# wtaylor17/ImageCFGen-Pytorch

Hardware: AMD Instinct MI355X
Metric: ALI training images/sec (E+G+D step), MorphoMNIST bs=512/GPU (higher is better)
Workload: dtype f32; 1 GPU; image_scms/mnist.py ALI iteration (EG step + 2 D steps + diagnostics), MorphoMNIST 28x28x1 synthetic, bs=512/GPU, fp32 MFMA, mode=stepper+hipgraph; global_batch=512, parallelism=dp1

## Files before the change

imagecfgen-pytorch_amd/csrc/ali_common.h:

```cpp
#pragma once
#include <hip/hip_runtime.h>
#include <stdint.h>
#include <stdio.h>
#include <stdlib.h>
#include "../../include/ali_hip.h"

namespace ali {

void set_error(const char* fmt, ...);

inline int check_launch(const char* what) {
  hipError_t e = hipGetLastError();
  if (e != hipSuccess) {
    set_error("%s: %s", what, hipGetErrorString(e));
    return ALI_ERR_LAUNCH;
  }
  return ALI_OK;
}

struct Tuning {
  int bm, bn, splitk;
  long long wgrad_small;
  int wgrad_blocks, wgrad_scap;
  int no_first_wgrad;
  int no_order;
  int tile_m_scale;
  int wbm, wbn;
  int no_xcd;
  int no_s2_first;
  int no_dma16;
  int no_t1_mfma;
};
inline Tuning read_tuning() {
  {
    auto num = [](const char* name) -> long long { const char* e = getenv(name); return e ? atoll(e) : 0; };
    Tuning v;
    v.bm = (int)num("ALI_BM"); v.bn = (int)num("ALI_BN"); v.splitk = (int)num("ALI_SPLITK");
    v.wgrad_small = getenv("ALI_WGRAD_SMALL") ? num("ALI_WGRAD_SMALL") : -1;
    v.wgrad_blocks = (int)num("ALI_WGRAD_BLOCKS"); v.wgrad_scap = (int)num("ALI_WGRAD_SCAP");
    v.no_order = (int)num("ALI_NO_ORDER");
    v.no_first_wgrad = (int)num("ALI_NO_FIRST_WGRAD");
    v.tile_m_scale = (int)num("ALI_TILE_M_SCALE");
    v.wbm = (int)num("ALI_WBM"); v.wbn = (int)num("ALI_WBN");
    v.no_t1_mfma = (int)num("ALI_NO_T1_MFMA");
    v.no_xcd = (int)num("ALI_NO_XCD");
    v.no_s2_first = (int)num("ALI_NO_S2_FIRST");
    v.no_dma16 = (int)num("ALI_NO_DMA16");
    return v;
  }
}
inline Tuning& tuning_slot() {
  static Tuning t = read_tuning();
  return t;
}
inline const Tuning& tuning() { return tuning_slot(); }

using f32x4 = __attribute__((ext_vector_type(4))) float;
using f32x16 = __attribute__((ext_vector_type(16))) float;

constexpr int kMaxTaps = 28;
constexpr int kNumCU = 256;

constexpr size_t kWsReserved = ALI_WS_RESERVED;
inline void* ws_payload(void* ws) { return ws ? static_cast<char*>(ws) + kWsReserved : nullptr; }
inline size_t ws_payload_bytes(size_t bytes) { return bytes > kWsReserved ? bytes - kWsReserved : 0; }

__device__ __forceinline__ float apply_act(float v, int act, float slope) {
  if (act == ALI_ACT_LEAKY) return v > 0.f ? v : v * slope;
  if (act == ALI_ACT_TANH) return tanhf(v);
  return v;
}
__device__ __forceinline__ float act_grad_from_output(float y, int act, float slope) {
  if (act == ALI_ACT_LEAKY) return y > 0.f ? 1.f : slope;
  if (act == ALI_ACT_TANH) return 1.f - y * y;
  return 1.f;
}

}
```

imagecfgen-pytorch_amd/csrc/gconv.hip:

```cpp
#include "ali_common.h"
#include <algorithm>
#include <vector>
#include <stdarg.h>
#include <stdlib.h>
#include <string.h>
#include <type_traits>

namespace ali {

static thread_local char g_err[512] = "";
void set_error(const char* fmt, ...) {
  va_list ap;
  va_start(ap, fmt);
  vsnprintf(g_err, sizeof(g_err), fmt, ap);
  va_end(ap);
}
const char* get_error() { return g_err; }

constexpr int BK = 32;
constexpr int LDK = BK + 4;
constexpr int kMaxGrid = 5;

struct Phase {
  int Hq, Wq;
// ... 959 lines not shown
      for (int pix = m_lo / d.B; pix <= m_hi / d.B; ++pix) {
        const int qh = pix / P.Wq, qw = pix - qh * P.Wq;
        unsigned wbits = 0u;
        for (int is = 0; is < P.ns; ++is)
          if ((unsigned)(qw * P.mult + P.dw[is]) < (unsigned)d.Win) wbits |= 1u << is;
        for (int ir = 0; ir < P.nr; ++ir)
          if ((unsigned)(qh * P.mult + P.dh[ir]) < (unsigned)d.Hin) mask |= wbits << (ir * P.ns);
      }
      cost.push_back(__builtin_popcount(mask));
    }
  }
  return true;
}

struct GJobRec {
  uint64_t state;
  int variant;
  int gx, gy, gz;
  int cost;
  GDesc d;
};
static_assert(sizeof(GJobRec) <= sizeof(AliGemmJob), "AliGemmJob too small");

static int finalize_and_launch(GDesc& d, void* ws, size_t ws_bytes, hipStream_t stream, bool vec, bool dense_k,
                               AliGemmJob* job = nullptr) {
  TileCfg tc;
  int max_taps = 0;
  const bool uni = vec && (d.Cin % BK) == 0;
  const bool dma_ok = d.f16 && uni && d.in16 && d.w16 && (d.Cin % 64) == 0 && !d.ep.bn_part && d.ep.in_ld <= 0 &&
                      tuning().no_dma16 == 0 && tuning().splitk == 0;
  const int tiles = plan_tiles(d, vec, tc, max_taps, dma_ok);
  if (tiles < 0) return ALI_ERR_BAD_ARG;
  const bool dma = tc.bm == 256;
  const int max_nkt = (max_taps * d.Cin + BK - 1) / BK;
  const bool pow2 = vec && (d.Cin == 4 || d.Cin == 8 || d.Cin == 16) && max_taps <= kMaxTaps;
  if (d.ep.bn_part) {
    const AliEpilogue& e = d.ep;
    bool ok = (e.bn_mode == 1 || e.bn_mode == 2) && !e.dact_y;
    if (e.bn_mode == 2) ok = ok && !e.mask && e.bn_x && e.bn_mean && e.bn_invstd && e.bn_groups <= 1;
    if (e.bn_mode == 1 && e.bn_groups > 1) {
      ok = ok && d.nphase == 1 && d.B % e.bn_groups == 0;
      const long long rows_g = (long long)(d.B / e.bn_groups) * (d.ph[0].pixmajor ? 1 : d.ph[0].Hq * d.ph[0].Wq);
      ok = ok && rows_g % tc.bm == 0 && (!d.ph[0].pixmajor || d.B % tc.bm == 0);
    }
    if (!ok) { set_error("gconv: bad fused BatchNorm epilogue (see AliEpilogue / ali_conv_mtiles)"); return ALI_ERR_BAD_ARG; }
    if (e.bn_slots > 0 && e.bn_slots != tiles) {
      set_error("gconv: bn_part was sized for %d slots, this launch has %d M-tiles (stale ali_conv_mtiles result?)", e.bn_slots, tiles);
      return ALI_ERR_BAD_ARG;
    }
  }
  const int ntile_n = (d.Cout + tc.bn - 1) / tc.bn;
  d.ldi = d.Cin;
  if (d.ep.in_ld > 0 || d.ep.out_ld > 0) {
    if ((d.ep.in_ld > 0 && (d.ep.in_ld < d.Cin || (vec && d.ep.in_ld % 4))) ||
        (d.ep.out_ld > 0 && (d.ep.out_ld < d.Cout || d.ep.bn_part))) {
      set_error("gconv: bad in_ld / out_ld (>= the channel count, in_ld % 4 == 0 for vector gathers, no out_ld with fused BatchNorm)");
      return ALI_ERR_BAD_ARG;
    }
    if (d.ep.in_ld > 0) d.ldi = d.ep.in_ld;
    if (d.ep.out_ld > 0) d.ldo = d.ep.out_ld;
  }
  d.out_elems = (long long)d.B * d.Hout * d.Wout * d.ldo;
  const long long in_elems = ((long long)d.B * d.Hin * d.Win - 1) * d.ldi + d.Cin;
  const long long w_elems = (long long)d.Cout * d.ldw;
  if (d.out_elems >= (1LL << 31) || in_elems >= (1LL << 30) || w_elems >= (1LL << 29)) {
    set_error("gconv: tensor too large for 32-bit byte offsets");
    return ALI_ERR_BAD_ARG;
  }
  d.in_bytes = (unsigned)(in_elems * 4);
  d.w_bytes = (unsigned)(w_elems * 4);
  int S = 1;
  const long long blocks = (long long)tiles * ntile_n;
  if (blocks < 2 * kNumCU && max_nkt >= 8 && dense_k) {
    static const double eff[5] = {1.0, 0.82, 0.96, 0.99, 1.0};
    double best = 1e30;
    for (int sc = 1; sc <= 8 && max_nkt / sc >= 4; ++sc) {
      if (sc > 1 && (size_t)sc * d.out_elems * sizeof(float) > ws_payload_bytes(ws_bytes)) break;
      const long long n = (blocks * sc + kNumCU - 1) / kNumCU;
      const double cost = (double)n / sc / eff[n < 4 ? n : 4] * max_nkt + (sc > 1 ? 0.5 * sc : 0.0);
      if (cost < 0.97 * best) { best = cost; S = sc; }
    }
  } else if (blocks < 2 * kNumCU && max_nkt >= 8) {
    S = (int)((2 * kNumCU + blocks - 1) / blocks);
    if (S > max_nkt / 4) S = max_nkt / 4;
    if (S > 32) S = 32;
    while (S > 1 && (size_t)S * d.out_elems * sizeof(float) > ws_payload_bytes(ws_bytes)) --S;
    if (S < 1) S = 1;
  }
  if (tuning().splitk > 0 && (size_t)tuning().splitk * d.out_elems * sizeof(float) <= ws_payload_bytes(ws_bytes))
    S = tuning().splitk;
  if (dma) S = 1;
  if (blocks > (long long)(kWsReserved / sizeof(int)) || !ws) S = 1;
  while (S > 1 && (long long)S * d.out_elems * 4 >= 0xFF000000LL) --S;
  d.splitk = S;
  d.kt_per_split = (max_nkt + S - 1) / S;
  if (d.kt_per_split < 1) d.kt_per_split = 1;
  d.ntile_m = tiles;
  d.ntile_n = ntile_n;
  d.tail_split = 1;
  d.tail_u0 = 0;
  if (S == 1 && uni && ws && blocks > kNumCU && blocks < 4 * kNumCU && blocks <= (long long)(kWsReserved / sizeof(int))
      && tuning().splitk == 0 && !dma) {
    const int R = (int)(blocks % kNumCU);
    int Sr = 1;
    while (R > 0 && Sr * 2 <= 8 && Sr * 2 * R <= kNumCU && max_nkt / (Sr * 2) >= 4) Sr *= 2;
    if (Sr > 1 && (size_t)Sr * d.out_elems * sizeof(float) <= ws_payload_bytes(ws_bytes) &&
        (long long)Sr * d.out_elems * 4 < 0xFF000000LL) {
      d.tail_split = Sr;
      d.tail_u0 = (int)(blocks - R);
    }
  }
  d.order = nullptr;
  if (d.ep.tile_order && uni && S == 1 && d.ep.tile_order_n == tiles && tuning().no_order == 0)
    d.order = reinterpret_cast<const int*>(d.ep.tile_order);
  d.lin1d = (d.tail_split > 1 || d.order) ? 1 : 0;
  if (d.tail_split == 1) d.tail_u0 = (int)blocks;
  d.xcd_chunk = 0;
  bool img_major = d.nphase >= 1;
  for (int i = 0; i < d.nphase; ++i) img_major = img_major && !d.ph[i].pixmajor;
  if (!d.lin1d && S == 1 && !job && img_major && blocks >= 8LL * kNumCU && blocks < (1LL << 30) && tuning().no_xcd == 0) {
    d.xcd_chunk = (int)((blocks + 7) / 8);
    d.lin1d = 1;
  }
  d.ctr = reinterpret_cast<int*>(ws);
  d.ws = reinterpret_cast<float*>(ws_payload(ws));
  dim3 grid(tiles, ntile_n, S), block(256);
  if (d.lin1d) grid = dim3(d.tail_u0 + (int)(blocks - d.tail_u0) * d.tail_split, 1, 1);
  if (d.xcd_chunk) grid = dim3(8 * d.xcd_chunk, 1, 1);
  if (tiles == 0 || d.out_elems == 0) return ALI_OK;
  const bool f16 = d.f16 && uni;
  const bool op16 = f16 && d.in16 && d.w16 && (d.Cin % 64) == 0;
  if (!d.f16) d.out16 = nullptr;
  if (job && uni && !f16 && ((tc.bm == 64 && tc.bn == 64) || (tc.bm == 128 && tc.bn == 32))) {
    GJobRec r;
    memset(&r, 0, sizeof(r));
    r.state = 1;
    r.variant = tc.bm == 64 ? 0 : 1;
    r.gx = (int)grid.x; r.gy = (int)grid.y; r.gz = (int)grid.z;
    r.cost = (max_nkt + S - 1) / S;
    r.d = d;
    memcpy(job, &r, sizeof(r));
    return ALI_OK;
  }
#define LAUNCH(BM_, BN_, WMM, WNN)                                                                    \
  do {                                                                                                  \
    if (op16) hipLaunchKernelGGL((gconv_kernel<BM_, BN_, WMM, WNN, 2, 2>), grid, block, 0, stream, d);  \
    else if (f16) hipLaunchKernelGGL((gconv_kernel<BM_, BN_, WMM, WNN, 2, 1>), grid, block, 0, stream, d); \
    else if (uni) hipLaunchKernelGGL((gconv_kernel<BM_, BN_, WMM, WNN, 2>), grid, block, 0, stream, d); \
    else if (pow2) hipLaunchKernelGGL((gconv_kernel<BM_, BN_, WMM, WNN, 3>), grid, block, 0, stream, d);  \
    else if (vec) hipLaunchKernelGGL((gconv_kernel<BM_, BN_, WMM, WNN, 1>), grid, block, 0, stream, d); \
    else hipLaunchKernelGGL((gconv_kernel<BM_, BN_, WMM, WNN, 0>), grid, block, 0, stream, d);          \
  } while (0)
  if (dma) {
    if (tc.bn != 256 || !op16) { set_error("gconv: no kernel for this tile"); return ALI_ERR_BAD_ARG; }
    block = dim3(512);
    hipLaunchKernelGGL((gconv_kernel512<256, 256, 2, 4, 2, 3>), grid, block, 0, stream, d);
    return check_launch("gconv_kernel512");
  }
  if (tc.bm > 128 || tc.bn > 128) { set_error("gconv: no kernel for this tile"); return ALI_ERR_BAD_ARG; }
  else if (tc.bm == 128 && tc.bn == 128) LAUNCH(128, 128, 2, 2);
  else if (tc.bm == 128 && tc.bn == 64) LAUNCH(128, 64, 2, 2);
  else if (tc.bm == 128 && tc.bn == 32) LAUNCH(128, 32, 4, 1);
  else if (tc.bm == 64 && tc.bn == 128) LAUNCH(64, 128, 2, 2);
  else LAUNCH(64, 64, 2, 2);
#undef LAUNCH
  return check_launch("gconv_kernel");
}

static bool geom_ok(const AliConvGeom* g) {
  if (!g) return false;
  if (g->B <= 0 || g->H <= 0 || g->W <= 0 || g->C <= 0 || g->P <= 0 || g->Q <= 0 || g->K <= 0) return false;
  if (g->R <= 0 || g->S <= 0 || g->R > kMaxGrid || g->S > kMaxGrid || g->stride <= 0 || g->pad < 0) return false;
  if (g->pad > 100) return false;
  return true;
}

static void fill_epilogue(GDesc& d, const AliEpilogue* ep) {
  if (ep) d.ep = *ep;
  else memset(&d.ep, 0, sizeof(d.ep));
  d.f16 = d.ep.mfma_f16 != 0;
  d.in16 = reinterpret_cast<const _Float16*>(d.ep.in16);
  d.w16 = reinterpret_cast<const _Float16*>(d.ep.w16);
  d.out16 = reinterpret_cast<_Float16*>(d.ep.out16);
}

}

using namespace ali;

extern "C" const char* ali_last_error(void) { return ali::get_error(); }
extern "C" int ali_version(void) { return 1; }
extern "C" void ali_reload_tuning(void) { ali::tuning_slot() = ali::read_tuning(); }

extern "C" size_t ali_conv_workspace_bytes(const AliConvGeom* g, int32_t which) {
  if (!geom_ok(g)) return 0;
  if (which == 0) return kWsReserved + (size_t)32 * g->B * g->P * g->Q * g->K * sizeof(float);
  if (which == 1) return kWsReserved + (size_t)32 * g->B * g->H * g->W * g->C * sizeof(float);
  return kWsReserved + (size_t)64 * g->R * g->S * g->C * g->K * sizeof(float);
}


constexpr int CF_C = 8, CF_K = 32;
constexpr int CF_PIXLD = 12;

struct CFDesc {
  const float* in; const float* w; float* out;
  AliEpilogue ep;
  int B, H, W, P, Q, R, S;
};

template <int TAPS, int CL = 8>
__global__ __launch_bounds__(256) void conv_first_kernel(const CFDesc d) {
  extern __shared__ __attribute__((aligned(16))) float cf_smem[];
  float* img = cf_smem;
  float* red = cf_smem + d.H * d.W * CF_PIXLD;
  const float* wl = d.w;
  const int t = threadIdx.x, lane = t & 63, wave = t >> 6;
  const int b = blockIdx.x;
  const int HW = d.H * d.W, PQ = d.P * d.Q;
  const float* src = d.in + (long long)b * HW * CF_C;
  for (int i = t; i < HW * 2; i += 256) {
    const f32x4 v = *reinterpret_cast<const f32x4*>(src + i * 4);
    *reinterpret_cast<f32x4*>(img + (i >> 1) * CF_PIXLD + (i & 1) * 4) = v;
  }
  const int lrow = lane & 31, lh = lane >> 5;
  constexpr int CF_WLD = TAPS * CF_C;
  constexpr int KL = TAPS * CL, NS = (KL + 1) / 2;
  f32x4 wf[CL == 8 ? TAPS : 1];
  float wb[CL == 8 ? 1 : NS];
  int aoff[CL == 8 ? 1 : NS];
  if constexpr (CL == 8) {
#pragma unroll
    for (int tp = 0; tp < TAPS; ++tp) wf[tp] = *reinterpret_cast<const f32x4*>(wl + lrow * CF_WLD + tp * CF_C + lh * 4);
  } else {
#pragma unroll
    for (int st = 0; st < NS; ++st) {
      const int k = 2 * st + lh;
      const bool live = k < KL;
      const int kk = live ? k : KL - 1;
      const int tp = kk / CL, c = kk - tp * CL;
      const int r = tp / d.S, sx = tp - r * d.S;
      wb[st] = live ? wl[lrow * CF_WLD + tp * CF_C + c] : 0.f;
      aoff[st] = (r * d.W + sx) * CF_PIXLD + c;
    }
  }
  __syncthreads();
  const AliEpilogue& ep = d.ep;
  const float bias = ep.bias ? ep.bias[lrow] : 0.f;
  const float smask = (ep.bn_part && ep.bn_stat_mask) ? ep.bn_stat_mask[(long long)b * ep.bn_mask_ld + lrow] : 1.f;
  float bs0 = 0.f, bs1 = 0.f;
  const int ntile = (PQ + 31) / 32;
  float* outb = d.out + (long long)b * PQ * CF_K;
  for (int mt = wave; mt < ntile; mt += 4) {
    const int m = mt * 32 + lrow;
    const int mc = m < PQ ? m : PQ - 1;
    const int p = mc / d.Q, q = mc - p * d.Q;
    f32x16 acc;
#pragma unroll
    for (int r = 0; r < 16; ++r) acc[r] = 0.f;
    if constexpr (CL == 8) {
      const float* a0 = img + (p * d.W + q) * CF_PIXLD + lh * 4;
#pragma unroll
      for (int tp = 0; tp < TAPS; ++tp) {
        const int r = tp / d.S, sx = tp - r * d.S;
        const f32x4 av = *reinterpret_cast<const f32x4*>(a0 + (r * d.W + sx) * CF_PIXLD);
#pragma unroll
        for (int e = 0; e < 4; ++e) acc = __builtin_amdgcn_mfma_f32_32x32x2f32(av[e], wf[tp][e], acc, 0, 0, 0);
      }
    } else {
      const float* a0 = img + (p * d.W + q) * CF_PIXLD;
#pragma unroll
      for (int st = 0; st < NS; ++st) {
        float av = a0[aoff[st]];
        if ((KL & 1) && st == NS - 1 && lh) av = 0.f;
        acc = __builtin_amdgcn_mfma_f32_32x32x2f32(av, wb[st], acc, 0, 0, 0);
      }
    }
#pragma unroll
    for (int r = 0; r < 16; ++r) {
      const int row = mt * 32 + (r & 3) + 8 * (r >> 2) + 4 * lh;
      if (row < PQ) {
        const float v = apply_act(acc[r] + bias, ep.act, ep.slope);
        outb[(long long)row * CF_K + lrow] = v;
        const float vs = v * smask;
        bs0 += vs;
        bs1 += vs * vs;
      }
    }
  }
  if (ep.bn_part) {
    bs0 += __shfl_xor(bs0, 32, 64);
    bs1 += __shfl_xor(bs1, 32, 64);
    if (lane < 32) { red[(0 * 4 + wave) * 32 + lane] = bs0; red[(1 * 4 + wave) * 32 + lane] = bs1; }
    __syncthreads();
    if (t < 32) {
      const float a = ((red[t] + red[32 + t]) + red[64 + t]) + red[96 + t];
      const float c = ((red[128 + t] + red[160 + t]) + red[192 + t]) + red[224 + t];
      ep.bn_part[((long long)0 * CF_K + t) * d.B + b] = a;
      ep.bn_part[((long long)1 * CF_K + t) * d.B + b] = c;
    }
  }
}

static bool conv_first_ok(const AliConvGeom* g, const AliEpilogue* ep, bool f16) {
  if (g->C != CF_C || g->K != CF_K || g->stride != 1 || g->pad != 0 || g->R != g->S || (g->R != 5 && g->R != 3)) return false;
  if (g->H > 32 || g->W > 32 || g->B < 64 || f16) return false;
  if (g->P != g->H - g->R + 1 || g->Q != g->W - g->S + 1) return false;
  if (ep && (ep->mask || ep->dact_y || (ep->bn_part && ep->bn_mode != 1))) return false;
  if (ep && ep->bn_part && ep->bn_groups > 1 && g->B % ep->bn_groups != 0) return false;
  return true;
}

static int conv_first_launch(const AliConvGeom* g, const float* x, const float* w, float* y, const AliEpilogue* ep,
                             hipStream_t stream) {
  CFDesc d;
  memset(&d, 0, sizeof(d));
  d.in = x; d.w = w; d.out = y;
  if (ep) d.ep = *ep;
  d.B = g->B; d.H = g->H; d.W = g->W; d.P = g->P; d.Q = g->Q; d.R = g->R; d.S = g->S;
  const size_t lds = ((size_t)g->H * g->W * CF_PIXLD + 256) * sizeof(float);
  const int live = ep ? ep->in_ch_live : 0;
  if (g->R == 5 && live == 5) hipLaunchKernelGGL((conv_first_kernel<25, 5>), dim3(g->B), dim3(256), lds, stream, d);
  else if (g->R == 5) hipLaunchKernelGGL((conv_first_kernel<25>), dim3(g->B), dim3(256), lds, stream, d);
  else hipLaunchKernelGGL((conv_first_kernel<9>), dim3(g->B), dim3(256), lds, stream, d);
  return check_launch("conv_first_kernel");
}

struct S2Desc {
  const float* in; const float* w; const float* bias; float* out; _Float16* out16;
  int B, H, W, P, Q, pad, act; float slope;
  unsigned in_bytes;
};

template <int C, bool F16>
__global__ __launch_bounds__(256) void conv_s2_first_kernel(const S2Desc d) {
  constexpr int T = 25, K = 64;
  constexpr int NP = F16 ? (C == 4 ? 7 : 13) : (C == 4 ? 13 : 25);
  constexpr int NBATCH = F16 ? NP : 13;
  constexpr int TPAD = F16 ? (C == 4 ? 28 : 26) : T;
  constexpr int LDW = F16 ? TPAD * C + 8 : T * C + (C == 8 ? 4 : 0);
  extern __shared__ __attribute__((aligned(16))) float s2_w[];
  _Float16* s2_h = reinterpret_cast<_Float16*>(s2_w);
  const int t = threadIdx.x, lane = t & 63, wave = t >> 6;
  if (F16) {
    for (int i = t; i < K * TPAD * C / 4; i += 256) {
      const int n = i / (TPAD * C / 4), rem = i - n * (TPAD * C / 4);
      f32x4 v = f32x4{0.f, 0.f, 0.f, 0.f};
      if (rem * 4 < T * C) v = *reinterpret_cast<const f32x4*>(d.w + (long long)n * T * C + rem * 4);
      f16x4 hv;
#pragma unroll
      for (int e = 0; e < 4; ++e) hv[e] = (_Float16)v[e];
      *reinterpret_cast<f16x4*>(s2_h + ((n >> 1) + 32 * (n & 1)) * LDW + rem * 4) = hv;
    }
  } else {
    for (int i = t; i < K * T * C / 4; i += 256) {
      const int n = i / (T * C / 4), rem = i - n * (T * C / 4);
      *reinterpret_cast<f32x4*>(s2_w + ((n >> 1) + 32 * (n & 1)) * LDW + rem * 4) =
          *reinterpret_cast<const f32x4*>(d.w + (long long)n * T * C + rem * 4);
    }
  }
  __syncthreads();
  const int m = lane & 31, h = lane >> 5;
  const int prow = blockIdx.x * 4 + wave;
  const int b = blockIdx.y;
  if (prow >= d.P) return;
  const __amdgpu_buffer_rsrc_t rin = __builtin_amdgcn_make_buffer_rsrc((void*)d.in, 0, d.in_bytes, 0x00020000);
  constexpr unsigned OOB = 0xFFFFFF00u;
  const float bias0 = d.bias ? d.bias[2 * m] : 0.f, bias1 = d.bias ? d.bias[2 * m + 1] : 0.f;
  const int ih0 = prow * 2 - d.pad;
  float* orow = d.out + ((long long)(b * d.P + prow) * d.Q) * K;
  _Float16* orow16 = d.out16 ? d.out16 + ((long long)(b * d.P + prow) * d.Q) * K : nullptr;
  for (int q0 = 0; q0 < d.Q; q0 += 32) {
    const int q = q0 + m;
    const int iw0 = q * 2 - d.pad;
    int wsel = 0;
    asm volatile("" : "+v"(wsel));
    f32x16 acc0, acc1;
#pragma unroll
    for (int r = 0; r < 16; ++r) { acc0[r] = 0.f; acc1[r] = 0.f; }
    auto gather = [&](int tap, int choff) -> f32x4 {
      const int r = tap / 5, sx = tap - r * 5;
      const int ih = ih0 + r, iw = iw0 + sx;
      const bool ok = tap < T && q < d.Q && (unsigned)ih < (unsigned)d.H && (unsigned)iw < (unsigned)d.W;
      const unsigned off = ok ? (unsigned)((((b * d.H + ih) * d.W + iw) * C + choff) * 4) : OOB;
      return __builtin_bit_cast(f32x4, __builtin_amdgcn_raw_buffer_load_b128(rin, (int)off, 0, 0));
    };
    if constexpr (F16) {
      const _Float16* wl = s2_h + m * LDW + wsel;
      f32x4 a[NP][2];
#pragma unroll
      for (int j = 0; j < NP; ++j) {
        if (C == 4) { a[j][0] = gather(4 * j + 2 * h, 0); a[j][1] = gather(4 * j + 2 * h + 1, 0); }
        else { a[j][0] = gather(2 * j + h, 0); a[j][1] = gather(2 * j + h, 4); }
      }
#pragma unroll
      for (int j = 0; j < NP; ++j) {
        f16x8 ha;
#pragma unroll
        for (int e = 0; e < 4; ++e) { ha[e] = (_Float16)a[j][0][e]; ha[4 + e] = (_Float16)a[j][1][e]; }
        const f16x8 w0 = *reinterpret_cast<const f16x8*>(wl + 16 * j + 8 * h);
        const f16x8 w1 = *reinterpret_cast<const f16x8*>(wl + 32 * LDW + 16 * j + 8 * h);
        acc0 = __builtin_amdgcn_mfma_f32_32x32x16_f16(ha, w0, acc0, 0, 0, 0);
        acc1 = __builtin_amdgcn_mfma_f32_32x32x16_f16(ha, w1, acc1, 0, 0, 0);
      }
    } else {
      const float* wl = s2_w + m * LDW + wsel;
#pragma unroll
      for (int j0 = 0; j0 < NP; j0 += NBATCH) {
        f32x4 a[NBATCH];
#pragma unroll
        for (int jj = 0; jj < NBATCH; ++jj) {
          const int j = j0 + jj;
          if (j >= NP) break;
          a[jj] = gather(C == 4 ? 2 * j + h : j, C == 8 ? 4 * h : 0);
        }
#pragma unroll
        for (int jj = 0; jj < NBATCH; ++jj) {
          const int j = j0 + jj;
          if (j >= NP) break;
          const int tap = C == 4 ? 2 * j + h : j;
          const int woff = (tap < T ? tap : 0) * C + (C == 8 ? 4 * h : 0);
          f32x4 w0 = *reinterpret_cast<const f32x4*>(wl + woff);
          f32x4 w1 = *reinterpret_cast<const f32x4*>(wl + 32 * LDW + woff);
          if (tap >= T) { w0 = f32x4{0.f, 0.f, 0.f, 0.f}; w1 = w0; }
#pragma unroll
          for (int e = 0; e < 4; ++e) {
            acc0 = __builtin_amdgcn_mfma_f32_32x32x2f32(a[jj][e], w0[e], acc0, 0, 0, 0);
            acc1 = __builtin_amdgcn_mfma_f32_32x32x2f32(a[jj][e], w1[e], acc1, 0, 0, 0);
          }
        }
      }
    }
#pragma unroll
    for (int r = 0; r < 16; ++r) {
      const int qq = q0 + (r & 3) + 8 * (r >> 2) + 4 * h;
      if (qq < d.Q) {
        const float v0 = apply_act(acc0[r] + bias0, d.act, d.slope), v1 = apply_act(acc1[r] + bias1, d.act, d.slope);
        *reinterpret_cast<float2*>(orow + (long long)qq * K + 2 * m) = float2{v0, v1};
        if (orow16) {
          using f16x2 = __attribute__((ext_vector_type(2))) _Float16;
          *reinterpret_cast<f16x2*>(orow16 + (long long)qq * K + 2 * m) = f16x2{(_Float16)v0, (_Float16)v1};
        }
      }
    }
  }
}

static bool conv_s2_first_ok(const AliConvGeom* g, const AliEpilogue* ep) {
  if (tuning().no_s2_first) return false;
  if ((g->C != 4 && g->C != 8) || g->K != 64 || g->R != 5 || g->S != 5 || g->stride != 2 || g->pad > 2) return false;
  if (g->P != (g->H + 2 * g->pad - 5) / 2 + 1 || g->Q != (g->W + 2 * g->pad - 5) / 2 + 1 || g->Q < 32 || g->B > 65535) return false;
  if ((long long)g->B * g->H * g->W * g->C >= (1LL << 29)) return false;
  if (ep && (ep->mask || ep->dact_y || ep->bn_part || ep->in_ld || ep->out_ld || ep->tile_order_n < 0)) return false;
  return true;
}

static int conv_s2_first_launch(const AliConvGeom* g, const float* x, const float* w, float* y, const AliEpilogue* ep,
                                hipStream_t stream) {
  S2Desc d;
  memset(&d, 0, sizeof(d));
  d.in = x; d.w = w; d.out = y;
  if (ep) { d.bias = ep->bias; d.act = ep->act; d.slope = ep->slope; if (ep->mfma_f16) d.out16 = reinterpret_cast<_Float16*>(ep->out16); }
  d.B = g->B; d.H = g->H; d.W = g->W; d.P = g->P; d.Q = g->Q; d.pad = g->pad;
  d.in_bytes = (unsigned)((long long)g->B * g->H * g->W * g->C * 4);
  dim3 grid((g->P + 3) / 4, g->B);
  const bool f16 = ep && ep->mfma_f16;
  if (g->C == 4 && f16) hipLaunchKernelGGL((conv_s2_first_kernel<4, true>), grid, dim3(256), (size_t)64 * 120 * sizeof(_Float16), stream, d);
  else if (g->C == 4) hipLaunchKernelGGL((conv_s2_first_kernel<4, false>), grid, dim3(256), (size_t)64 * 100 * sizeof(float), stream, d);
  else if (f16) hipLaunchKernelGGL((conv_s2_first_kernel<8, true>), grid, dim3(256), (size_t)64 * 216 * sizeof(_Float16), stream, d);
  else hipLaunchKernelGGL((conv_s2_first_kernel<8, false>), grid, dim3(256), (size_t)64 * 204 * sizeof(float), stream, d);
  return check_launch("conv_s2_first_kernel");
}

static void setup_fwd(const AliConvGeom* g, GDesc& d) {
  d.B = g->B; d.Hin = g->H; d.Win = g->W; d.Cin = g->C;
  d.Hout = g->P; d.Wout = g->Q; d.Cout = g->K; d.ldo = g->K;
  d.ldw = g->R * g->S * g->C;
  d.S = g->S;
  d.nphase = 1;
  Phase& P = d.ph[0];
  P.Hq = g->P; P.Wq = g->Q; P.oh0 = 0; P.ow0 = 0; P.ostep = 1; P.mult = g->stride;
  P.M = g->B * g->P * g->Q;
  P.nr = g->R; P.ns = g->S;
  for (int r = 0; r < g->R; ++r) { P.dh[r] = (signed char)(r - g->pad); P.wr[r] = (unsigned char)r; }
  for (int s = 0; s < g->S; ++s) { P.dw[s] = (signed char)(s - g->pad); P.ws[s] = (unsigned char)s; }
}

static bool setup_bwd_data(const AliConvGeom* g, GDesc& d) {
  d.B = g->B; d.Hin = g->P; d.Win = g->Q; d.Cin = g->K;
  d.Hout = g->H; d.Wout = g->W; d.Cout = g->C; d.ldo = g->C;
  d.ldw = g->R * g->S * g->K;
  d.S = g->S;
  const int st = g->stride;
  if (st > 2) { set_error("ali_conv_bwd_data: stride %d unsupported", st); return false; }
  d.nphase = 0;
  for (int ph = 0; ph < st; ++ph)
    for (int pw = 0; pw < st; ++pw) {
      const int Hq = (g->H - ph + st - 1) / st, Wq = (g->W - pw + st - 1) / st;
      if (Hq <= 0 || Wq <= 0) continue;
      Phase& P = d.ph[d.nphase++];
      P.Hq = Hq; P.Wq = Wq; P.oh0 = ph; P.ow0 = pw; P.ostep = st; P.mult = 1;
      P.M = g->B * Hq * Wq;
      P.nr = P.ns = 0;
      for (int r = 0; r < g->R; ++r) {
        const int nh = ph + g->pad - r;
        if (((nh % st) + st) % st) continue;
        P.dh[P.nr] = (signed char)(nh / st);
        P.wr[P.nr] = (unsigned char)r;
        ++P.nr;
      }
      for (int s = 0; s < g->S; ++s) {
        const int nw = pw + g->pad - s;
        if (((nw % st) + st) % st) continue;
        P.dw[P.ns] = (signed char)(nw / st);
        P.ws[P.ns] = (unsigned char)s;
        ++P.ns;
      }
    }
  return true;
}

extern "C" int32_t ali_conv_mtiles(const AliConvGeom* g, int32_t which, int32_t mfma_f16, int32_t* tile_rows,
                                   int32_t* pixel_major) {
  if (!geom_ok(g) || (which != 0 && which != 1)) return 0;
  if (which == 0 && conv_first_ok(g, nullptr, mfma_f16 != 0)) {
    if (tile_rows) *tile_rows = g->P * g->Q;
    if (pixel_major) *pixel_major = 0;
    return g->B;
  }
  GDesc d;
  memset(&d, 0, sizeof(d));
  d.f16 = mfma_f16 != 0;
  bool vec;
  if (which == 0) { setup_fwd(g, d); vec = (g->C % 4) == 0; }
  else { if (!setup_bwd_data(g, d)) return 0; vec = (g->K % 4) == 0; }
  TileCfg tc;
  int max_taps = 0;
  const int tiles = plan_tiles(d, vec, tc, max_taps);
  if (tiles < 0) return 0;
  if (tile_rows) *tile_rows = tc.bm;
  if (pixel_major) *pixel_major = d.ph[0].pixmajor;
  return tiles;
}

extern "C" int32_t ali_conv_tile_order(const AliConvGeom* g, int32_t which, int32_t mfma_f16, int32_t* order,
                                       int32_t cap) {
  if (!geom_ok(g) || (which != 0 && which != 1) || !order) return 0;
  if (which == 0 && conv_first_ok(g, nullptr, mfma_f16 != 0)) return 0;
  GDesc d;
  memset(&d, 0, sizeof(d));
  d.f16 = mfma_f16 != 0;
  bool vec;
  if (which == 0) { setup_fwd(g, d); vec = (g->C % 4) == 0; }
  else { if (!setup_bwd_data(g, d)) return 0; vec = (g->K % 4) == 0; }
  if (!vec || (d.Cin % BK) != 0) return 0;
  TileCfg tc;
  int max_taps = 0;
  const int tiles = plan_tiles(d, vec, tc, max_taps);
  if (tiles <= 0 || tiles > cap) return 0;
  std::vector<int> cost;
  if (!tile_costs(d, tc.bm, cost) || (int)cost.size() != tiles) return 0;
  if (*std::max_element(cost.begin(), cost.end()) == *std::min_element(cost.begin(), cost.end())) return 0;
  std::vector<int> idx(tiles);
  for (int i = 0; i < tiles; ++i) idx[i] = i;
  std::stable_sort(idx.begin(), idx.end(), [&](int a, int b) { return cost[a] > cost[b]; });
  const int nt = (d.Cout + tc.bn - 1) / tc.bn;
  const long long blocks = (long long)tiles * nt;
  bool tail_split = false;
  if (blocks > kNumCU && blocks < 4 * kNumCU) {
    const int R = (int)(blocks % kNumCU);
    const int max_nkt = (max_taps * d.Cin + BK - 1) / BK;
    tail_split = R > 0 && 2 * R <= kNumCU && max_nkt / 2 >= 4;
  }
  const int W = std::min(tiles, 4 * kNumCU / nt);
  if (tail_split || W < 2) {
    for (int i = 0; i < tiles; ++i) order[i] = idx[i];
    return tiles;
  }
  const int full = (tiles / 8) * 8;
  auto slot_of = [&](int r, int by) { return r < full ? (r / 8) * 8 * nt + by * 8 + (r % 8) : full * nt + (r - full) * nt + by; };
  std::vector<long long> load(kNumCU, 0);
  std::vector<char> used(W, 0);
  for (int i = 0; i < W; ++i) {
    const int tile = idx[i];
    int best = -1;
    long long best_load = 0;
    for (int p = 0; p < W; ++p) {
      if (used[p]) continue;
      long long l = 0;
      for (int by = 0; by < nt; ++by) l = std::max(l, load[slot_of(p, by) % kNumCU]);
      if (best < 0 || l < best_load) { best = p; best_load = l; }
    }
    used[best] = 1;
    order[best] = tile;
    for (int by = 0; by < nt; ++by) load[slot_of(best, by) % kNumCU] += cost[tile];
  }
  for (int i = W; i < tiles; ++i) order[i] = idx[i];
  return tiles;
}

extern "C" int32_t ali_conv_writes_out16(const AliConvGeom* g, int32_t which) {
  (void)which;
  return geom_ok(g) ? 1 : 0;
}

extern "C" int32_t ali_conv_uses_f16(const AliConvGeom* g, int32_t which, const AliEpilogue* ep) {
  if (!geom_ok(g) || !ep || !ep->mfma_f16) return 0;
  if (which == 0 && conv_s2_first_ok(g, ep)) return 1;
  return ((which == 0 ? g->C : g->K) % 32) == 0 ? 1 : 0;
}

static int conv_fwd_impl(const AliConvGeom* g, const float* x, const float* w, float* y, const AliEpilogue* ep,
                         void* ws, size_t ws_bytes, ali_stream_t stream, AliGemmJob* job) {
  if (!geom_ok(g) || !x || !w || !y) { set_error("ali_conv_fwd: bad argument"); return ALI_ERR_BAD_ARG; }
  if (conv_first_ok(g, nullptr, ep && ep->mfma_f16)) {
    if (conv_first_ok(g, ep, false)) {
      if (ep && ep->bn_part && ep->bn_slots > 0 && ep->bn_slots != g->B) {
        set_error("ali_conv_fwd: bn_part was sized for %d slots, the per-image kernel leaves %d", ep->bn_slots, g->B);
        return ALI_ERR_BAD_ARG;
      }
      return conv_first_launch(g, x, w, y, ep, (hipStream_t)stream);
    }
    if (ep && ep->bn_part) { set_error("ali_conv_fwd: epilogue not supported for this first-layer geometry"); return ALI_ERR_BAD_ARG; }
  }
  if (conv_s2_first_ok(g, ep)) return conv_s2_first_launch(g, x, w, y, ep, (hipStream_t)stream);
  GDesc d;
  memset(&d, 0, sizeof(d));
  d.in = x; d.w = w; d.out = y;
// ... 81 lines not shown
```

Measured before the change: 79690 images/s.

## Make first-layer conv kernel persistent with register-prefetched next image

Replaces the one-block-per-image first conv launch with a persistent grid capped at a few blocks per CU. Each block loops over images, loads weights into registers once, and prefetches the next image into registers while computing the current one. This amortizes weight loads and hides global-load latency. The cost is higher register pressure, which can lower occupancy, plus an extra barrier per image. An env var can switch back to the old kernel.

```diff
diff --git a/imagecfgen-pytorch_amd/csrc/ali_common.h b/imagecfgen-pytorch_amd/csrc/ali_common.h
--- a/imagecfgen-pytorch_amd/csrc/ali_common.h
+++ b/imagecfgen-pytorch_amd/csrc/ali_common.h
@@ -30,6 +30,8 @@
   int no_s2_first;
   int no_dma16;
   int no_t1_mfma;
+  int no_cf_persist;
+  int cf_blocks_per_cu;
 };
 inline Tuning read_tuning() {
   {
@@ -46,6 +48,8 @@
     v.no_xcd = (int)num("ALI_NO_XCD");
     v.no_s2_first = (int)num("ALI_NO_S2_FIRST");
     v.no_dma16 = (int)num("ALI_NO_DMA16");
+    v.no_cf_persist = (int)num("ALI_NO_CF_PERSIST");
+    v.cf_blocks_per_cu = (int)num("ALI_CF_BLOCKS_PER_CU");
     return v;
   }
 }
diff --git a/imagecfgen-pytorch_amd/csrc/gconv.hip b/imagecfgen-pytorch_amd/csrc/gconv.hip
--- a/imagecfgen-pytorch_amd/csrc/gconv.hip
+++ b/imagecfgen-pytorch_amd/csrc/gconv.hip
@@ -1285,6 +1285,137 @@
   }
 }
 
+constexpr int kCfBlocksPerCU = 2;
+
+template <int TAPS, int CL = 8>
+__global__ __launch_bounds__(256) void conv_first_kernel_persist(const CFDesc d) {
+  extern __shared__ __attribute__((aligned(16))) float cf_smem[];
+  constexpr int S = TAPS == 25 ? 5 : 3;
+  const int HW = d.H * d.W, PQ = d.P * d.Q;
+  float* img = cf_smem;
+  float* red = cf_smem + HW * CF_PIXLD;
+  const float* wl = d.w;
+  const int t = threadIdx.x, lane = t & 63, wave = t >> 6;
+  constexpr int NPF = 8;
+  f32x4 pf[NPF];
+  auto fetch = [&](int b) {
+    const float* src = d.in + (long long)b * HW * CF_C;
+#pragma unroll
+    for (int j = 0; j < NPF; ++j) {
+      const int i = t + 256 * j;
+      pf[j] = i < HW * 2 ? *reinterpret_cast<const f32x4*>(src + i * 4) : f32x4{0.f, 0.f, 0.f, 0.f};
+    }
+  };
+  auto stash = [&]() {
+#pragma unroll
+    for (int j = 0; j < NPF; ++j) {
+      const int i = t + 256 * j;
+      if (i < HW * 2) *reinterpret_cast<f32x4*>(img + (i >> 1) * CF_PIXLD + (i & 1) * 4) = pf[j];
+    }
+  };
+  fetch(blockIdx.x);
+  const int lrow = lane & 31, lh = lane >> 5;
+  constexpr int CF_WLD = TAPS * CF_C;
+  constexpr int KL = TAPS * CL, NS = (KL + 1) / 2;
+  f32x4 wf[CL == 8 ? TAPS : 1];
+  float wb[CL == 8 ? 1 : NS];
+  int aoff[CL == 8 ? 1 : NS];
+  if constexpr (CL == 8) {
+#pragma unroll
+    for (int tp = 0; tp < TAPS; ++tp) wf[tp] = *reinterpret_cast<const f32x4*>(wl + lrow * CF_WLD + tp * CF_C + lh * 4);
+  } else {
+#pragma unroll
+    for (int st = 0; st < NS; ++st) {
+      const int k = 2 * st + lh;
+      const bool live = k < KL;
+      const int kk = live ? k : KL - 1;
+      const int tp = kk / CL, c = kk - tp * CL;
+      const int r = tp / S, sx = tp - r * S;
+      wb[st] = live ? wl[lrow * CF_WLD + tp * CF_C + c] : 0.f;
+      aoff[st] = (r * d.W + sx) * CF_PIXLD + c;
+    }
+  }
+  stash();
+  __syncthreads();
+  const AliEpilogue& ep = d.ep;
+  const float bias = ep.bias ? ep.bias[lrow] : 0.f;
+  const int ntile = (PQ + 31) / 32;
+  for (int b = blockIdx.x; b < d.B; b += gridDim.x) {
+    const bool more = b + (int)gridDim.x < d.B;
+    if (more) fetch(b + gridDim.x);
+    const float smask = (ep.bn_part && ep.bn_stat_mask) ? ep.bn_stat_mask[(long long)b * ep.bn_mask_ld + lrow] : 1.f;
+    float bs0 = 0.f, bs1 = 0.f;
+    float* outb = d.out + (long long)b * PQ * CF_K;
+    for (int mt = wave; mt < ntile; mt += 4) {
+      const int m = mt * 32 + lrow;
+      const int mc = m < PQ ? m : PQ - 1;
+      const int p = mc / d.Q, q = mc - p * d.Q;
+      f32x16 acc;
+#pragma unroll
+      for (int r = 0; r < 16; ++r) acc[r] = 0.f;
+      if constexpr (CL == 8) {
+        const float* a0 = img + (p * d.W + q) * CF_PIXLD + lh * 4;
+#pragma unroll
+        for (int tp = 0; tp < TAPS; ++tp) {
+          const int r = tp / S, sx = tp - r * S;
+          const f32x4 av = *reinterpret_cast<const f32x4*>(a0 + (r * d.W + sx) * CF_PIXLD);
+#pragma unroll
+          for (int e = 0; e < 4; ++e) acc = __builtin_amdgcn_mfma_f32_32x32x2f32(av[e], wf[tp][e], acc, 0, 0, 0);
+        }
+      } else {
+        const float* a0 = img + (p * d.W + q) * CF_PIXLD;
+        constexpr int CH = 16, NCH = (NS + CH - 1) / CH;
+        float ab[2][CH];
+#pragma unroll
+        for (int j = 0; j < CH; ++j)
+          if (j < NS) ab[0][j] = a0[aoff[j]];
+#pragma unroll
+        for (int c = 0; c < NCH; ++c) {
+#pragma unroll
+          for (int j = 0; j < CH; ++j)
+            if ((c + 1) * CH + j < NS) ab[(c + 1) & 1][j] = a0[aoff[(c + 1) * CH + j]];
+          __builtin_amdgcn_sched_barrier(0);
+#pragma unroll
+          for (int j = 0; j < CH; ++j) {
+            const int st = c * CH + j;
+            if (st < NS) {
+              float av = ab[c & 1][j];
+              if ((KL & 1) && st == NS - 1 && lh) av = 0.f;
+              acc = __builtin_amdgcn_mfma_f32_32x32x2f32(av, wb[st], acc, 0, 0, 0);
+            }
+          }
+          __builtin_amdgcn_sched_barrier(0);
+        }
+      }
+#pragma unroll
+      for (int r = 0; r < 16; ++r) {
+        const int row = mt * 32 + (r & 3) + 8 * (r >> 2) + 4 * lh;
+        if (row < PQ) {
+          const float v = apply_act(acc[r] + bias, ep.act, ep.slope);
+          outb[(long long)row * CF_K + lrow] = v;
+          const float vs = v * smask;
+          bs0 += vs;
+          bs1 += vs * vs;
+        }
+      }
+    }
+    __syncthreads();
+    if (more) stash();
+    if (ep.bn_part) {
+      bs0 += __shfl_xor(bs0, 32, 64);
+      bs1 += __shfl_xor(bs1, 32, 64);
+      if (lane < 32) { red[(0 * 4 + wave) * 32 + lane] = bs0; red[(1 * 4 + wave) * 32 + lane] = bs1; }
+    }
+    __syncthreads();
+    if (ep.bn_part && t < 32) {
+      const float a = ((red[t] + red[32 + t]) + red[64 + t]) + red[96 + t];
+      const float c = ((red[128 + t] + red[160 + t]) + red[192 + t]) + red[224 + t];
+      ep.bn_part[((long long)0 * CF_K + t) * d.B + b] = a;
+      ep.bn_part[((long long)1 * CF_K + t) * d.B + b] = c;
+    }
+  }
+}
+
 static bool conv_first_ok(const AliConvGeom* g, const AliEpilogue* ep, bool f16) {
   if (g->C != CF_C || g->K != CF_K || g->stride != 1 || g->pad != 0 || g->R != g->S || (g->R != 5 && g->R != 3)) return false;
   if (g->H > 32 || g->W > 32 || g->B < 64 || f16) return false;
@@ -1303,10 +1434,19 @@
   d.B = g->B; d.H = g->H; d.W = g->W; d.P = g->P; d.Q = g->Q; d.R = g->R; d.S = g->S;
   const size_t lds = ((size_t)g->H * g->W * CF_PIXLD + 256) * sizeof(float);
   const int live = ep ? ep->in_ch_live : 0;
-  if (g->R == 5 && live == 5) hipLaunchKernelGGL((conv_first_kernel<25, 5>), dim3(g->B), dim3(256), lds, stream, d);
-  else if (g->R == 5) hipLaunchKernelGGL((conv_first_kernel<25>), dim3(g->B), dim3(256), lds, stream, d);
-  else hipLaunchKernelGGL((conv_first_kernel<9>), dim3(g->B), dim3(256), lds, stream, d);
-  return check_launch("conv_first_kernel");
+  if (tuning().no_cf_persist) {
+    if (g->R == 5 && live == 5) hipLaunchKernelGGL((conv_first_kernel<25, 5>), dim3(g->B), dim3(256), lds, stream, d);
+    else if (g->R == 5) hipLaunchKernelGGL((conv_first_kernel<25>), dim3(g->B), dim3(256), lds, stream, d);
+    else hipLaunchKernelGGL((conv_first_kernel<9>), dim3(g->B), dim3(256), lds, stream, d);
+    return check_launch("conv_first_kernel");
+  }
+  int per_cu = tuning().cf_blocks_per_cu;
+  if (per_cu < 1 || per_cu > 8) per_cu = kCfBlocksPerCU;
+  const dim3 grid(g->B < per_cu * kNumCU ? g->B : per_cu * kNumCU);
+  if (g->R == 5 && live == 5) hipLaunchKernelGGL((conv_first_kernel_persist<25, 5>), grid, dim3(256), lds, stream, d);
+  else if (g->R == 5) hipLaunchKernelGGL((conv_first_kernel_persist<25>), grid, dim3(256), lds, stream, d);
+  else hipLaunchKernelGGL((conv_first_kernel_persist<9>), grid, dim3(256), lds, stream, d);
+  return check_launch("conv_first_kernel_persist");
 }
 
 struct S2Desc {
```

Result: no change. 79990 images/s, median of 6 (+0.4%).
